# OpenHardware-Initiative/Drone-OA-IREE-ViT-Accelerator

Measured on AMD Instinct MI355X. Metric: frames/s on ITAViTLSTM int8, 60x90 depth input, higher is better.
Workload: dtype int8+f32; 1 GPU; ITAViTLSTM int8 end-to-end forward (BASELINE config 4): 1024 synthetic 60x90 depth frames per GPU per step, LSTM state carried, velocity all-gather; frames_per_gpu=1024, global_batch=1024, parallelism=dp1, image_dtype=u8, weights=seed-0 synthetic QAT (tests/golden), gather_every=1, gather=none (one GPU), schedule=one stream

## Files before the change

### drone-oa-iree-vit-accelerator_amd/csrc/ita_f16x3_kernels.h

```cpp
#pragma once
#include <type_traits>
#include "ita_device.h"

typedef _Float16 f16x8 __attribute__((ext_vector_type(8)));
typedef _Float16 f16x4 __attribute__((ext_vector_type(4)));
typedef float f32x16 __attribute__((ext_vector_type(16)));
typedef unsigned u32x2 __attribute__((ext_vector_type(2)));
typedef unsigned u32x4 __attribute__((ext_vector_type(4)));

__device__ __forceinline__ __amdgpu_buffer_rsrc_t ita_rsrc(const void* p) {
  return __builtin_amdgcn_make_buffer_rsrc(const_cast<void*>(p), (short)0, 0x7FFFFFFF, 0x00020000);
}
constexpr int ITA_SC1 = 16;

__device__ __forceinline__ void split_f16(float x, _Float16& hi, _Float16& lo) {
  hi = (_Float16)x;
  lo = (_Float16)(x - (float)hi);
}

struct ItaGemmSplitArgs {
  const _Float16 *a_hi, *a_lo; int lda;
  const _Float16 *w_hi, *w_lo; int ldw;
  float* out;
  int M, N, K;
// ... 51 lines not shown
  for (int i = 0; i < TM; ++i)
#pragma unroll
    for (int j = 0; j < TN; ++j)
#pragma unroll
      for (int e = 0; e < 16; ++e) acc[i][j][e] = 0.0f;

  auto stage = [&](int buf, int t) {
    char* b = lds + buf * L::BUF;
    const int k0 = kbeg + t * 64;
    const int m0s = (g.dbg & 16) ? 0 : m0, n0s = (g.dbg & 32) ? 0 : n0, k0s = (g.dbg & 64) ? t * 64 : k0;
    stage_plane<BM, NT>(g.a_hi, g.lda, m0s, g.M - 1, k0s, b, tid);
    stage_plane<BM, NT>(g.a_lo, g.lda, m0s, g.M - 1, k0s, b + L::A_PLANE, tid);
    stage_plane<BN, NT>(g.w_hi, g.ldw, n0s, g.N - 1, k0s, b + 2 * L::A_PLANE, tid);
    stage_plane<BN, NT>(g.w_lo, g.ldw, n0s, g.N - 1, k0s, b + 2 * L::A_PLANE + L::W_PLANE, tid);
  };

  auto compute = [&](int buf) {
    const char* b = lds + buf * L::BUF;
    const char *ah = b, *al = b + L::A_PLANE, *wh = b + 2 * L::A_PLANE, *wl = wh + L::W_PLANE;
#pragma unroll
    for (int ks = 0; ks < 4; ++ks) {
      f16x8 fah[TM], fal[TM], fwh[TN], fwl[TN];
#pragma unroll
      for (int i = 0; i < TM; ++i) {
        const int row = wm * (BM / WM) + i * 32 + r;
        fah[i] = frag_f16(ah, row, 2 * ks + h);
        fal[i] = frag_f16(al, row, 2 * ks + h);
      }
#pragma unroll
      for (int j = 0; j < TN; ++j) {
        const int row = wn * (BN / WN) + j * 32 + r;
        fwh[j] = frag_f16(wh, row, 2 * ks + h);
        fwl[j] = frag_f16(wl, row, 2 * ks + h);
      }
#pragma unroll
      for (int i = 0; i < TM; ++i)
#pragma unroll
        for (int j = 0; j < TN; ++j) {
          acc[i][j] = __builtin_amdgcn_mfma_f32_32x32x16_f16(fal[i], fwh[j], acc[i][j], 0, 0, 0);
          acc[i][j] = __builtin_amdgcn_mfma_f32_32x32x16_f16(fah[i], fwl[j], acc[i][j], 0, 0, 0);
          acc[i][j] = __builtin_amdgcn_mfma_f32_32x32x16_f16(fah[i], fwh[j], acc[i][j], 0, 0, 0);
        }
    }
  };
  int cur = 0;
  stage(0, 0);
  __syncthreads();
  for (int t = 0; t < nt; ++t) {
    if (t + 1 < nt && !(g.dbg & 2)) stage(cur ^ 1, t + 1);
    if (!(g.dbg & 1)) compute(g.dbg & 8 ? 0 : cur);
    if (!(g.dbg & 4)) __syncthreads();
    cur ^= 1;
  }
  float* out = g.out + (size_t)zsplit * g.M * g.N;
#pragma unroll
  for (int i = 0; i < TM; ++i)
#pragma unroll
    for (int j = 0; j < TN; ++j) {
      const int n = n0 + wn * (BN / WN) + j * 32 + r;
#pragma unroll
      for (int e = 0; e < 16; ++e) {
        const int m = m0 + wm * (BM / WM) + i * 32 + (e & 3) + 8 * (e >> 2) + 4 * h;
        if (m < g.M) __hip_atomic_store(out + (size_t)m * g.N + n, acc[i][j][e], __ATOMIC_RELAXED, __HIP_MEMORY_SCOPE_AGENT);
      }
    }
}

constexpr int ITA_GEMM_SMALL_NSTG = 3;
constexpr int ita_gemm_small_lds(int mt) { return ITA_GEMM_SMALL_NSTG * (2 * mt + 2) * 32 * 128; }
constexpr int ita_waitcnt_vm(int n) { return (n & 15) | ((n >> 4) << 14) | 0x0F70; }
template <int MT>
__global__ __launch_bounds__(256) void ita_gemm_f16x3_small_kernel(const ItaGemmSplitArgs g) {
  constexpr int NSTG = ITA_GEMM_SMALL_NSTG, PLANE = 32 * 128, APL = MT * PLANE, STG = 2 * APL + 2 * PLANE;
  constexpr int DMA = 2 * MT + 2;
  static_assert(NSTG == 3 && DMA < 64, "one younger k-tile in flight at the wait; vmcnt range");
  extern __shared__ __attribute__((aligned(16))) char lds[];
  const int tid = threadIdx.x, lane = tid & 63, wave = __builtin_amdgcn_readfirstlane(tid >> 6), r = lane & 31, h = lane >> 5;
  const int z = blockIdx.x % g.nsplit, n0 = (blockIdx.x / g.nsplit) * 32, m0 = blockIdx.y * 32 * MT;
  const int kslice = g.K / g.nsplit, kbeg = z * kslice, nt = kslice / 64;
  auto stage = [&](int kt, int slot) {
    char* b = lds + slot * STG;
    const int k0 = kbeg + kt * 64;
    stage_plane<32 * MT, 256>(g.a_hi, g.lda, m0, g.M - 1, k0, b, tid);
    stage_plane<32 * MT, 256>(g.a_lo, g.lda, m0, g.M - 1, k0, b + APL, tid);
    stage_plane<32, 256>(g.w_hi, g.ldw, n0, g.N - 1, k0, b + 2 * APL, tid);
    stage_plane<32, 256>(g.w_lo, g.ldw, n0, g.N - 1, k0, b + 2 * APL + PLANE, tid);
  };
#pragma unroll
  for (int s = 0; s < NSTG - 1; ++s)
    if (s < nt) stage(s, s);
  f32x16 acc;
#pragma unroll
  for (int e = 0; e < 16; ++e) acc[e] = 0.0f;
  const bool compute = wave < MT && m0 + 32 * wave < g.M;
  for (int kt = 0; kt < nt; ++kt) {
    if (kt + 1 < nt) __builtin_amdgcn_s_waitcnt(ita_waitcnt_vm(DMA)); else __builtin_amdgcn_s_waitcnt(ita_waitcnt_vm(0));
    __builtin_amdgcn_s_waitcnt(0xC07F);
    __builtin_amdgcn_s_barrier();
    asm volatile("" ::: "memory");
    __builtin_amdgcn_sched_barrier(0);
    if (kt + NSTG - 1 < nt) stage(kt + NSTG - 1, (kt + NSTG - 1) % NSTG);
    if (compute) {
      const char* b = lds + (kt % NSTG) * STG;
      const char *pah = b + wave * PLANE, *pal = b + APL + wave * PLANE, *pwh = b + 2 * APL, *pwl = pwh + PLANE;
#pragma unroll
      for (int ks = 0; ks < 4; ++ks) {
        const f16x8 ah = frag_f16(pah, r, 2 * ks + h), al = frag_f16(pal, r, 2 * ks + h);
        const f16x8 wh = frag_f16(pwh, r, 2 * ks + h), wl = frag_f16(pwl, r, 2 * ks + h);
        acc = __builtin_amdgcn_mfma_f32_32x32x16_f16(al, wh, acc, 0, 0, 0);
        acc = __builtin_amdgcn_mfma_f32_32x32x16_f16(ah, wl, acc, 0, 0, 0);
        acc = __builtin_amdgcn_mfma_f32_32x32x16_f16(ah, wh, acc, 0, 0, 0);
      }
    }
  }
  if (!compute) return;
  float* out = g.out + (size_t)z * g.M * g.N;
#pragma unroll
  for (int e = 0; e < 16; ++e) {
// ... 31 lines not shown
    }
  }
  float* out = g.out + (size_t)z * g.M * g.N;
#pragma unroll
  for (int e = 0; e < 16; ++e) {
    const int m = m0 + (e & 3) + 8 * (e >> 2) + 4 * h;
    if (m < g.M) out[(size_t)m * g.N + n0 + r] = acc[e];
  }
}

__device__ __forceinline__ size_t ita_lstm_plane_index(int b, int k) {
  return ((size_t)(((b >> 5) * 4 + (k >> 6)) * 4 + ((k >> 4) & 3)) * 64 + ((k >> 3) & 1) * 32 + (b & 31)) * 8 + (k & 7);
}
__device__ __forceinline__ float lstm_sigmoid_fast(float x) {
  return __builtin_amdgcn_rcpf(1.0f + __builtin_amdgcn_exp2f(x * -1.44269504088896341f));
}
__device__ __forceinline__ float lstm_tanh_fast(float x) {
  return 1.0f - 2.0f * __builtin_amdgcn_rcpf(__builtin_amdgcn_exp2f(x * 2.88539008177792681f) + 1.0f);
}
struct ItaLstmHeadArgs {
  const float* part; float inv_fold_scale;
  const _Float16 *w0_hi, *w0_lo; float inv_wscale0;
  const float* bias0;
  const _Float16 *w1_hi, *w1_lo, *w2_hi, *w2_lo;
  float inv_wscale1, inv_wscale2;
  const float *bsum1, *bsum2;
  const float *desvel, *quat;
  const float *h_in, *c_in;
  float *h_out, *c_out;
  size_t lstride;
  _Float16 *p1_hi, *p1_lo, *p2_hi, *p2_lo;
  const float *fc_w, *fc_b; float* vel;
  unsigned *cnt, *err;
  int B;
  const int* slots;
};
constexpr int ITA_HEAD_CNT_STRIDE = 64;
constexpr unsigned ITA_HEAD_ERR_TIMEOUT = 1;
constexpr unsigned long long ITA_HEAD_SPIN_TICKS = 200000000ull;
__device__ __forceinline__ f16x8 ita_load_sc1_f16x8(const _Float16* base, int byte_off) {
  return __builtin_bit_cast(f16x8, __builtin_amdgcn_raw_buffer_load_b128(ita_rsrc(base), byte_off, 0, ITA_SC1));
}
__device__ __forceinline__ bool ita_head_poll(unsigned* cnt, unsigned target, unsigned* err) {
  const unsigned long long t0 = wall_clock64();
  while (__hip_atomic_load(cnt, __ATOMIC_RELAXED, __HIP_MEMORY_SCOPE_AGENT) < target) {
    if (wall_clock64() - t0 > ITA_HEAD_SPIN_TICKS) {
      __hip_atomic_fetch_or(err, ITA_HEAD_ERR_TIMEOUT, __ATOMIC_RELAXED, __HIP_MEMORY_SCOPE_AGENT);
      return false;
    }
    __builtin_amdgcn_s_sleep(2);
  }
  return true;
}
template <int NS>
__global__ __launch_bounds__(256, 2) void ita_lstm_head_kernel(const ItaLstmHeadArgs a) {
  __shared__ __attribute__((aligned(16))) float big[32 * 132 + 32 * 36];
  __shared__ __attribute__((aligned(16))) f16x8 hin[2][2][4][2][64];
  __shared__ __attribute__((aligned(16))) _Float16 pub[2][32][8];
  __shared__ unsigned flag;
  float (*hs)[132] = (float (*)[132])big;
  float (*pt)[36] = (float (*)[36])(big + 32 * 132);
  float (*part)[16][64] = (float (*)[16][64])big;
  const int tid = threadIdx.x, lane = tid & 63, wave = __builtin_amdgcn_readfirstlane(tid >> 6);
  const int ft = blockIdx.x >> 4, ut = blockIdx.x & 15, f0 = ft * 32;
  const int r = lane & 31, h = lane >> 5;
  const int B = a.B;
  const int ef = tid >> 3, eu = tid & 7;
  int rh[4], rb0 = min(f0 + r, B - 1), reb = min(f0 + ef, B - 1);
#pragma unroll
  for (int i = 0; i < 4; ++i) rh[i] = min(f0 + 2 * (4 * wave + i) + h, B - 1);
  if (a.slots) {
#pragma unroll
    for (int i = 0; i < 4; ++i) rh[i] = a.slots[rh[i]];
    rb0 = a.slots[rb0];
    reb = a.slots[reb];
  }

  f32x4 pz[NS];
#pragma unroll
  for (int z = 0; z < NS; ++z)
    pz[z] = *(const f32x4*)(a.part + ((size_t)z * B + min(f0 + 8 * wave + (lane >> 3), B - 1)) * 512 + ut * 32 + 4 * (lane & 7));
  f32x4 hv[4];
#pragma unroll
  for (int i = 0; i < 4; ++i) hv[i] = *(const f32x4*)(a.h_in + (size_t)rh[i] * 128 + 4 * r);
  const int b0 = f0 + r, u0 = ut * 8 + 4 * h;
  const size_t sb0 = (size_t)rb0;
  if (wave >= 2) {
    f32x4 hx[2][4][2];
#pragma unroll
    for (int l = 0; l < 2; ++l)
#pragma unroll
      for (int s = 0; s < 4; ++s) {
        const float* src = a.h_in + (l + 1) * a.lstride + sb0 * 128 + 64 * (wave - 2) + 16 * s + 8 * h;
        hx[l][s][0] = *(const f32x4*)src;
        hx[l][s][1] = *(const f32x4*)(src + 4);
      }
    __builtin_amdgcn_sched_barrier(0);
#pragma unroll
    for (int l = 0; l < 2; ++l)
#pragma unroll
      for (int s = 0; s < 4; ++s) {
        f16x8 xh, xl;
#pragma unroll
        for (int j = 0; j < 8; ++j) {
          _Float16 hi, lo;
          split_f16(hx[l][s][j >> 2][j & 3], hi, lo);
          xh[j] = hi;
          xl[j] = lo;
        }
        hin[l][wave - 2][s][0][lane] = xh;
        hin[l][wave - 2][s][1][lane] = xl;
      }
  }
  f16x8 wh[9], wl[9];
  f32x4 q = {0.0f, 0.0f, 0.0f, 0.0f}, ci0 = {0.0f, 0.0f, 0.0f, 0.0f}, bz[4];
  float dv = 0.0f;
  if (wave == 0) {
    const _Float16* wfr_hi = a.w0_hi + ((size_t)ut * 9 * 64 + lane) * 8;
    const _Float16* wfr_lo = a.w0_lo + ((size_t)ut * 9 * 64 + lane) * 8;
#pragma unroll
    for (int s = 0; s < 9; ++s) {
      wh[s] = *(const f16x8*)(wfr_hi + s * 512);
      wl[s] = *(const f16x8*)(wfr_lo + s * 512);
    }
    const int bc = min(b0, B - 1);
    q = *(const f32x4*)(a.quat + (size_t)bc * 4);
    dv = a.desvel[bc];
    ci0 = *(const f32x4*)(a.c_in + sb0 * 128 + u0);
#pragma unroll
    for (int gt = 0; gt < 4; ++gt) bz[gt] = *(const f32x4*)(a.bias0 + gt * 128 + u0);
  }
  const size_t wo = ((size_t)((ut * 4 + wave) * 4) * 64 + lane) * 8;
  f16x8 w1h[4], w1l[4];
#pragma unroll
  for (int s = 0; s < 4; ++s) {
    w1h[s] = *(const f16x8*)(a.w1_hi + wo + 512 * s);
    w1l[s] = *(const f16x8*)(a.w1_lo + wo + 512 * s);
  }
  const int eb = f0 + ef, un = ut * 8 + eu;
  const size_t esb = (size_t)reb;
  const float c1_prev = a.c_in[a.lstride + esb * 128 + un], c2_prev = a.c_in[2 * a.lstride + esb * 128 + un];
  float bs1[4], bs2[4];
#pragma unroll
  for (int gt = 0; gt < 4; ++gt) {
    bs1[gt] = a.bsum1[gt * 128 + un];
    bs2[gt] = a.bsum2[gt * 128 + un];
  }
  __builtin_amdgcn_sched_barrier(0);
  {
    f32x4 ps = pz[0];
#pragma unroll
    for (int z = 1; z < NS; ++z) ps += pz[z];
    *(f32x4*)&pt[8 * wave + (lane >> 3)][4 * (lane & 7)] = ps;
  }
#pragma unroll
  for (int i = 0; i < 4; ++i) *(f32x4*)&hs[2 * (4 * wave + i) + h][4 * r] = hv[i];
  __syncthreads();

  f32x4 hn0 = {0.0f, 0.0f, 0.0f, 0.0f};
  if (wave == 0) {
    f32x16 acc;
#pragma unroll
    for (int e = 0; e < 16; ++e) acc[e] = 0.0f;
    f32x4 xlast0 = {0.0f, 0.0f, 0.0f, 0.0f};
    float xlast1 = 0.0f;
    if (h == 0) {
      xlast0 = (f32x4){dv / 10.0f, q.x, q.y, q.z};
      xlast1 = q.w;
    }
#pragma unroll
    for (int s = 0; s < 9; ++s) {
      f32x4 x0 = xlast0, x1 = {xlast1, 0.0f, 0.0f, 0.0f};
      if (s < 8) {
        x0 = *(const f32x4*)&hs[r][16 * s + 8 * h];
        x1 = *(const f32x4*)&hs[r][16 * s + 8 * h + 4];
      }
      f16x8 xh, xl;
#pragma unroll
      for (int j = 0; j < 8; ++j) {
        const float x = j < 4 ? x0[j & 3] : x1[j & 3];
        const _Float16 hi = (_Float16)x;
        xh[j] = hi;
        xl[j] = (_Float16)(x - (float)hi);
      }
      acc = __builtin_amdgcn_mfma_f32_32x32x16_f16(wl[s], xh, acc, 0, 0, 0);
      acc = __builtin_amdgcn_mfma_f32_32x32x16_f16(wh[s], xl, acc, 0, 0, 0);
      acc = __builtin_amdgcn_mfma_f32_32x32x16_f16(wh[s], xh, acc, 0, 0, 0);
    }
    f32x4 cn;
#pragma unroll
    for (int q = 0; q < 4; ++q) {
      float g[4];
#pragma unroll
      for (int gt = 0; gt < 4; ++gt)
        g[gt] = (pt[r][gt * 8 + 4 * h + q] * a.inv_fold_scale + acc[4 * gt + q] * a.inv_wscale0) + bz[gt][q];
      const float ig = lstm_sigmoid_fast(g[0]), fg = lstm_sigmoid_fast(g[1]), cg = lstm_tanh_fast(g[2]), og = lstm_sigmoid_fast(g[3]);
      const float c = fmaf(fg, ci0[q], ig * cg);
      cn[q] = c;
      hn0[q] = og * lstm_tanh_fast(c);
    }
    if (b0 < B) *(f32x4*)(a.c_out + sb0 * 128 + u0) = cn;
    f16x4 x_hi, x_lo;
#pragma unroll
    for (int q = 0; q < 4; ++q) {
      _Float16 x, y;
      split_f16(hn0[q], x, y); x_hi[q] = x; x_lo[q] = y;
    }
    const int o0 = (int)ita_lstm_plane_index(b0, u0) * 2;
    __builtin_amdgcn_raw_buffer_store_b64(__builtin_bit_cast(u32x2, x_hi), ita_rsrc(a.p1_hi), o0, 0, ITA_SC1);
    __builtin_amdgcn_raw_buffer_store_b64(__builtin_bit_cast(u32x2, x_lo), ita_rsrc(a.p1_lo), o0, 0, ITA_SC1);
  }
  asm volatile("s_waitcnt vmcnt(0)" ::: "memory");
  __syncthreads();
  if (tid == 0) __hip_atomic_fetch_add(a.cnt + ft * ITA_HEAD_CNT_STRIDE, 1u, __ATOMIC_RELAXED, __HIP_MEMORY_SCOPE_AGENT);
  f16x8 w2h[4], w2l[4];
#pragma unroll
  for (int s = 0; s < 4; ++s) {
    w2h[s] = *(const f16x8*)(a.w2_hi + wo + 512 * s);
    w2l[s] = *(const f16x8*)(a.w2_lo + wo + 512 * s);
  }

#pragma unroll
  for (int l = 1; l <= 2; ++l) {
    if (tid == 0) flag = ita_head_poll(a.cnt + ft * ITA_HEAD_CNT_STRIDE, 16u * l, a.err) ? 1u : 0u;
    __syncthreads();
    if (!flag) return;
    if (l == 1 && wave == 0 && b0 < B) *(f32x4*)(a.h_out + sb0 * 128 + u0) = hn0;
    f16x8 fah[4], fal[4];
    if (wave < 2) {
      const int ao = (((ft * 4 + wave) * 4) * 64 + lane) * 16;
      const _Float16* ph = l == 1 ? a.p1_hi : a.p2_hi;
      const _Float16* pl = l == 1 ? a.p1_lo : a.p2_lo;
#pragma unroll
      for (int s = 0; s < 4; ++s) {
        fah[s] = ita_load_sc1_f16x8(ph, ao + 1024 * s);
        fal[s] = ita_load_sc1_f16x8(pl, ao + 1024 * s);
      }
    } else {
#pragma unroll
      for (int s = 0; s < 4; ++s) {
        fah[s] = hin[l - 1][wave - 2][s][0][lane];
        fal[s] = hin[l - 1][wave - 2][s][1][lane];
      }
    }
    f32x16 acc;
#pragma unroll
    for (int e = 0; e < 16; ++e) acc[e] = 0.0f;
#pragma unroll
    for (int s = 0; s < 4; ++s) {
      const f16x8 fwh = l == 1 ? w1h[s] : w2h[s], fwl = l == 1 ? w1l[s] : w2l[s];
      acc = __builtin_amdgcn_mfma_f32_32x32x16_f16(fwl, fah[s], acc, 0, 0, 0);
      acc = __builtin_amdgcn_mfma_f32_32x32x16_f16(fwh, fal[s], acc, 0, 0, 0);
      acc = __builtin_amdgcn_mfma_f32_32x32x16_f16(fwh, fah[s], acc, 0, 0, 0);
    }
#pragma unroll
    for (int e = 0; e < 16; ++e) part[wave][e][lane] = acc[e];
    __syncthreads();
    float gsum[4];
    const int pl = ef + 32 * (eu >> 2);
#pragma unroll
    for (int gte = 0; gte < 4; ++gte) {
      const int e = 4 * gte + (eu & 3);
      gsum[gte] = ((part[0][e][pl] + part[1][e][pl]) + part[2][e][pl]) + part[3][e][pl];
    }
    const float iws = l == 1 ? a.inv_wscale1 : a.inv_wscale2;
    const float* bs = l == 1 ? bs1 : bs2;
    const float gi = gsum[0] * iws + bs[0], gf = gsum[1] * iws + bs[1], gg = gsum[2] * iws + bs[2], go = gsum[3] * iws + bs[3];
    const float ig = lstm_sigmoid_fast(gi), fg = lstm_sigmoid_fast(gf), cg = lstm_tanh_fast(gg), og = lstm_sigmoid_fast(go);
    const float c = fmaf(fg, l == 1 ? c1_prev : c2_prev, ig * cg);
    const float hn = og * lstm_tanh_fast(c);
    const size_t so = l * a.lstride + esb * 128 + un;
    if (eb < B) {
      a.c_out[so] = c;
      if (l == 1) a.h_out[so] = hn;
      else
        __builtin_amdgcn_raw_buffer_store_b32(__builtin_bit_cast(unsigned, hn), ita_rsrc(a.h_out), (int)(so * 4), 0, ITA_SC1);
    }
    if (l == 1) {
      _Float16 x, y;
      split_f16(hn, x, y);
      pub[0][ef][eu] = x;
      pub[1][ef][eu] = y;
      __syncthreads();
      if (wave == 0 && h == 0) {
        const int o = (int)ita_lstm_plane_index(f0 + r, ut * 8) * 2;
        const f16x8 vh = *(const f16x8*)&pub[0][r][0], vl = *(const f16x8*)&pub[1][r][0];
        __builtin_amdgcn_raw_buffer_store_b128(__builtin_bit_cast(u32x4, vh), ita_rsrc(a.p2_hi), o, 0, ITA_SC1);
        __builtin_amdgcn_raw_buffer_store_b128(__builtin_bit_cast(u32x4, vl), ita_rsrc(a.p2_lo), o, 0, ITA_SC1);
      }
    }
    asm volatile("s_waitcnt vmcnt(0)" ::: "memory");
    __syncthreads();
    if (tid == 0) {
      const unsigned prev = __hip_atomic_fetch_add(a.cnt + ft * ITA_HEAD_CNT_STRIDE, 1u, __ATOMIC_RELAXED, __HIP_MEMORY_SCOPE_AGENT);
      if (l == 2) flag = prev == 47u ? 1u : 0u;
    }
  }

  __syncthreads();
  if (!flag) return;
  if (tid == 0) __hip_atomic_store(a.cnt + ft * ITA_HEAD_CNT_STRIDE, 0u, __ATOMIC_RELAXED, __HIP_MEMORY_SCOPE_AGENT);
  float (*fw)[128] = (float (*)[128])(big + 32 * 132);
  int fro[4];
#pragma unroll
  for (int i = 0; i < 4; ++i) fro[i] = min(f0 + ((i * 256 + tid) >> 5), B - 1);
  if (a.slots) {
#pragma unroll
    for (int i = 0; i < 4; ++i) fro[i] = a.slots[fro[i]];
  }
  f32x4 hr[4];
#pragma unroll
  for (int i = 0; i < 4; ++i) {
    const int off = (int)((2 * a.lstride + (size_t)fro[i] * 128 + 4 * (tid & 31)) * 4);
    hr[i] = __builtin_bit_cast(f32x4, __builtin_amdgcn_raw_buffer_load_b128(ita_rsrc(a.h_out), off, 0, ITA_SC1));
  }
  const f32x4 wv = *(const f32x4*)(a.fc_w + 4 * min(tid, 95));
#pragma unroll
  for (int i = 0; i < 4; ++i) *(f32x4*)&hs[(i * 256 + tid) >> 5][4 * (tid & 31)] = hr[i];
  if (tid < 96) *(f32x4*)&fw[tid >> 5][4 * (tid & 31)] = wv;
  __syncthreads();
  if (tid < 96) {
    const int fr = tid / 3, o = tid - 3 * fr, b = f0 + fr;
    if (b < B) {
      float acc = a.fc_b[o];
      for (int k = 0; k < 128; ++k) acc = fmaf(hs[fr][k], fw[o][k], acc);
      a.vel[(size_t)b * 3 + o] = acc;
    }
  }
}

__global__ void ita_split_planes_kernel(const float* __restrict__ x, _Float16* __restrict__ hi, _Float16* __restrict__ lo,
                                        int width, int ld, int rows) {
  const size_t i8 = ((size_t)blockIdx.x * blockDim.x + threadIdx.x) * 8;
  if (i8 >= (size_t)rows * width) return;
  const size_t r = i8 / width, c = i8 - r * width;
  f16x8 vh, vl;
#pragma unroll
  for (int j = 0; j < 8; ++j) {
    _Float16 a, b;
    split_f16(x[i8 + j], a, b);
    vh[j] = a; vl[j] = b;
  }
  *(f16x8*)(hi + r * ld + c) = vh;
  *(f16x8*)(lo + r * ld + c) = vl;
}

__global__ void ita_impulse_kernel(float* x, int rows, int width, int col0) {
  const size_t idx = (size_t)blockIdx.x * blockDim.x + threadIdx.x;
  if (idx >= (size_t)rows * width) return;
  const int i = (int)(idx / width), c = (int)(idx % width);
  x[idx] = (c == col0 + i) ? 1.0f : 0.0f;
}

struct ItaTailBigArgs {
  const float* x;
  const _Float16 *w_hi, *w_lo;
  const float* bias;
  float inv_wscale;
  float* out;
  int B, E, TH, TW, CO, nchunk;
  int accumulate;
};
template <int NT, int WAVES, int TPS>
struct ItaTailBigLds {
  static constexpr int HP = (2 * WAVES + 2) * 34;
  static constexpr int A_PLANE = HP * 64;
  static constexpr int W_PLANE = TPS * NT * 16 * 64;
  static constexpr int AH = 0, AL = A_PLANE, WH = 2 * A_PLANE, WL = WH + W_PLANE;
  static constexpr int GEO_I = WL + W_PLANE;
  static constexpr int GEO_F = GEO_I + HP * 16;
  static constexpr int TOTAL = GEO_F + HP * 8;
};

template <int NT, int WAVES, int TPS>
__global__ __launch_bounds__(64 * WAVES) void ita_tail_big_kernel(const ItaTailBigArgs a) {
  using L = ItaTailBigLds<NT, WAVES, TPS>;
  static_assert(9 % TPS == 0, "taps per weight stage must divide 9");
  constexpr int W_CHUNK_HALVES = 9 * NT * 16 * 32;
  constexpr int NTHR = 64 * WAVES;
  extern __shared__ __attribute__((aligned(16))) char lds[];
  const int tid = threadIdx.x, lane = tid & 63, wave = tid >> 6;
// ... 484 lines not shown
```

### drone-oa-iree-vit-accelerator_amd/csrc/ita_stream_kernel.h

```cpp
#pragma once
#include "ita_int8_kernels.h"
#ifndef ITA_ABLATE
#define ITA_ABLATE 0
#endif

struct ItaStreamArgs {
  const char* image;
  const float* x;
  float* y;
  _Float16 *y_hi, *y_lo;
  int ld_planes;
  float* x1_tap;
  float inv_sx, mq, mk, mv, ml, mc, mo, so;
  float f_inv_sx, m1, m2, s2;
  int B;
  int fuse_ln;
  unsigned long long* stamps;
  const float* h0_src;
  float* h0_dst;
  const int* slots;
  const int8_t* xq;
  int8_t* yq;
  const void* img;
  float* tok_tap;
// ... 384 lines not shown
    const unsigned H1 = (unsigned)(8.0f * g.h1) & 7u, W1 = (unsigned)(32.0f * g.w1) & 31u, H0 = 8u - H1, W0 = 32u - W1;
    const unsigned w00 = (H0 * W0) & 255u, w01 = (H0 * W1) & 255u, w10 = (H1 * W0) & 255u, w11 = (H1 * W1) & 255u;
    __builtin_amdgcn_s_waitcnt(0xc07f);
    __builtin_amdgcn_wave_barrier();
    unsigned pb[13];
#pragma unroll
    for (int s = 0; s < 13; ++s) {
      if constexpr (ITA_ABLATE & 512) { pb[s] = w00 * s; continue; }
      const int off = tap[4 * s + kq];
      pb[s] = (unsigned)win[off] * w00 + (unsigned)win[off + 2] * w01 + (unsigned)win[off + 192] * w10 +
              (unsigned)win[off + 194] * w11;
    }
    tok_u8_fragments(pb, tk_a0, tk_a1);
  };
  auto tok_step = [&](int ct, int ol) {
    if constexpr (ITA_ABLATE & 1024) { tk_out[4 * ct] = __int_as_float(tk_a0[ct]); return; }
    float o4[4];
    tok_u8_tile<E>(lds + L::CW, ct, ol, ol >> 4, tk_a0, tk_a1, o4);
#pragma unroll
    for (int i = 0; i < 4; ++i) tk_out[4 * ct + i] = o4[i];
  };
  auto tok_finish = [&](int fb, bool store_tap, float (&xr)[EC], int ol) {
    const int qi = ol & 15, kq = ol >> 4, token = wave * 16 + qi;
#pragma unroll
    for (int i = 0; i < 16; ++i) xr[i] = tk_out[i];
    layernorm_q16<E>(xr, lnp + 4 * E, lnp + 5 * E, EC * kq);
    if (a.tok_tap && store_tap) {
      float* o = a.tok_tap + ((size_t)fb * S + token) * E + EC * kq;
#pragma unroll
      for (int i = 0; i < EC; i += 4) *(f32x4*)(o + i) = (f32x4){xr[i], xr[i + 1], xr[i + 2], xr[i + 3]};
    }
  };

  if (STAMP && a.stamps && (tid & 255) == 0)
    a.stamps[(((size_t)blockIdx.x * 8) * 2 + (wave >> 2)) * 16 + 12] = __builtin_amdgcn_s_memrealtime();
  float xr[EC];
  i32x4 xq_cur[NK];
  f32x4 h0_cur = {0.0f, 0.0f, 0.0f, 0.0f};
  int h0_row_next = 0;
  {
    int ol = lane;
    asm volatile("" : "+v"(ol));
    if constexpr (IO8) {
      const int8_t* xrow = a.xq + ((size_t)blockIdx.x * S + wave * 16 + (ol & 15)) * E + EC * (ol >> 4);
#pragma unroll
      for (int c = 0; c < NK; ++c) xq_cur[c] = *(const i32x4*)(xrow + 16 * c);
    } else if constexpr (TOK == 0) {
      ld_tok_items<E>(a.x + ((size_t)blockIdx.x * S + wave * 16 + (ol & 15)) * E, ol >> 4, xr);
    }
    if (a.h0_dst && tid < 32) {
      const size_t row = a.slots ? (size_t)a.slots[blockIdx.x] : (size_t)blockIdx.x;
      h0_cur = *(const f32x4*)(a.h0_src + row * 128 + 4 * tid);
    }
    constexpr int T0 = L::LNP / 16, NT = (L::IMAGE - L::LNP) / 16, NTJ = (NT + 511) / 512;
    constexpr int NW = L::LNP / 16, NWJ = (NW + 511) / 512;
    static_assert(L::LNP % 16 == 0, "");
    i32x4 vt[NTJ], vw[NWJ];
#pragma unroll
    for (int j = 0; j < NTJ; ++j) {
      const int p = tid + 512 * j;
      vt[j] = (i32x4){0, 0, 0, 0};
      if (p < NT) vt[j] = *(const i32x4*)(a.image + (size_t)(T0 + p) * 16);
    }
#pragma unroll
    for (int j = 0; j < NWJ; ++j) {
      const int p = tid + 512 * j;
      vw[j] = (i32x4){0, 0, 0, 0};
      if (p < NW) vw[j] = *(const i32x4*)(a.image + (size_t)p * 16);
    }
    if constexpr (TOK != 0) tok_fetch(blockIdx.x, ol);
    if (tid < 2 * P) colsum[tid] = ITA_ACC_BIAS;
#pragma unroll
    for (int j = 0; j < NTJ; ++j) {
      const int p = tid + 512 * j;
      if (p < NT) *(i32x4*)(lds + (T0 + p) * 16) = vt[j];
    }
#pragma unroll
    for (int j = 0; j < NWJ; ++j) {
      const int p = tid + 512 * j;
      if (p < NW) *(i32x4*)(lds + p * 16) = vw[j];
    }
    if constexpr (TOK != 0) tok_fill(ol);
    lds_barrier();
    if constexpr (TOK != 0) {
      tok_blend(ol);
#pragma unroll
      for (int ct = 0; ct < 4; ++ct) tok_step(ct, ol);
      tok_finish(blockIdx.x, true, xr, ol);
    }
    if constexpr (TOK == 0 && !IO8) tok_items_transpose<E>(xr);
  }
  if (STAMP && a.stamps && (tid & 255) == 0)
    a.stamps[(((size_t)blockIdx.x * 8) * 2 + (wave >> 2)) * 16 + 13] = __builtin_amdgcn_s_memrealtime();

  for (int b = blockIdx.x; b < a.B; b += gridDim.x, ++fi) {
    int ol = lane;
    asm volatile("" : "+v"(ol));
    const int qi = E > 64 ? (ol & 15) : qi0, kq = E > 64 ? (ol >> 4) : kq0, token = wave * 16 + qi;
    const int nb = b + gridDim.x;
    const bool more = nb < a.B;
    int* cs = colsum + (fi & 1) * P;
    ITA_SSTAMP(0);
    i32x4 xf[NK];
#pragma unroll
    for (int c = 0; c < NK; ++c) {
      if constexpr (IO8) {
        xf[c] = xq_cur[c];
      } else {
        unsigned p4[4];
        q_pack16(&xr[16 * c], a.inv_sx, p4);
        xf[c] = (i32x4){(int)p4[0], (int)p4[1], (int)p4[2], (int)p4[3]};
      }
    }
    if (!(ITA_ABLATE & 128) && a.h0_dst && tid < 32) {
      *(f32x4*)(a.h0_dst + (size_t)b * 128 + 4 * ol) = h0_cur;
      if (nb < a.B) h0_row_next = a.slots ? a.slots[nb] : nb;
    }

    i32x4 qf[3];
    {
      ItaFr<4 * NK> fr[2];
      i32x4 ac[3][4];
      auto load = [&](int g, ItaFr<4 * NK>& f, i32x4 (&acc)[4]) {
        const int mat = g / 3, t0 = 4 * (g - 3 * mat);
        if (mat == 0) ld_nat<NK, P>(f, acc, lds + L::WQ, l_bq, t0, qi, kq);
        else if (mat == 1) ld_nat<NK, P>(f, acc, lds + L::WK, l_bk, t0, qi, kq);
        else ld_natv<NK, P>(f, acc, lds + L::WV, (const int*)(lds + L::VB4), t0, qi, kq);
      };
      auto epilogue = [&](int g, const i32x4 (&acc)[4]) {
        const int mat = g / 3, gg = g - 3 * mat;
        if (mat == 0) {
          qf[gg] = rq_group(acc, a.mq, fq);
        } else if (mat == 1) {
          *(i32x4*)(lds + L::K + (((4 * gg + kq) * S + token) << 4)) = rq_group(acc, a.mk, fk);
        } else {
          const i32x4 p4 = rq_group(acc, a.mv, fv);
#pragma unroll
          for (int t = 0; t < 4; ++t) {
            const int d = (4 * gg + t) * 16 + qi;
            *(int*)(lds + L::VT + (((((wave >> 2) * 4 + kq) * P) + d) << 4) + 4 * (wave & 3)) = p4[t];
            atomicAdd(&cs[d], __builtin_amdgcn_sdot4(p4[t], 0x01010101, 0, false) << 7);
          }
// ... 385 lines not shown
```

### drone-oa-iree-vit-accelerator_amd/csrc/ita_plugin.hip

```cpp
#include <hip/hip_runtime.h>

#include <algorithm>
#include <cstdio>
#include <cstdlib>
#include <cstring>
#include <mutex>
#include <string>
#include <atomic>
#include <functional>
#include <thread>
#include <vector>

#include "../../include/ita_mi355x.h"
#include "../../include/ita_weights.h"
#include "../../include/ita_wire.h"
#include "ita_f16x3_kernels.h"
#include "ita_lstm_seq_kernel.h"
#include "ita_f32_kernels.h"
#include "ita_int8_kernels.h"
#include "ita_stream_kernel.h"
#include "ita_long_attn_kernel.h"
#include "ita_ffn_f32_kernel.h"
#include "ita_attn_f32_kernel.h"
#include "ita_ffn_f32_e128_kernel.h"
// ... 1206 lines not shown
  *status = 0;
  if (!h->head_sync) return ITA_OK;
  unsigned v = 0;
  HIPCHK(hipDeviceSynchronize());
  HIPCHK(hipMemcpy(&v, h->head_sync, sizeof(v), hipMemcpyDeviceToHost));
  if (v) {
    HIPCHK(hipMemset(h->head_sync, 0, h->head_sync_bytes));
    HIPCHK(hipDeviceSynchronize());
  }
  *status = (int)v;
  return ITA_OK;
}

int ita_get_attn_kind(ita_handle h, int layer, int* kind) {
  if (!h || !h->loaded) return fail(ITA_ERR_NO_WEIGHTS, "no weights loaded");
  if (!kind || layer < 0 || layer >= h->hdr.num_layers) return fail(ITA_ERR_INVALID_ARG, "bad pointer or layer");
  *kind = h->layers[layer].attn_f32 ? ITA_ATTN_F32 : ITA_ATTN_INT8;
  return ITA_OK;
}

int ita_mha_f32(ita_handle h, int layer, const float* x, float* y, int batch, void* stream) {
  int rc = check(h, batch);
  if (rc) return rc;
  if (!x || !y || layer < 0 || layer >= h->hdr.num_layers) return fail(ITA_ERR_INVALID_ARG, "bad pointer or layer");
  return launch_attn_f32(h, layer, x, y, batch, false, (hipStream_t)stream);
}

int ita_encoder_layer(ita_handle h, int layer, const float* x, float* y, int batch, void* stream) {
  int rc = check(h, batch);
  if (rc) return rc;
  if (!x || !y || layer < 0 || layer >= h->hdr.num_layers) return fail(ITA_ERR_INVALID_ARG, "bad pointer or layer");
  return launch_encoder(h, layer, x, y, nullptr, nullptr, nullptr, batch, (hipStream_t)stream);
}

int ita_debug_encoder_stamps(ita_handle h, int layer, const float* x, const void* image_u8, float* y, int batch,
                             unsigned long long* stamps, void* stream) {
  int rc = check(h, batch);
  if (rc) return rc;
  if ((!x && !image_u8) || !y || !stamps || layer < 0 || layer >= h->hdr.num_layers)
    return fail(ITA_ERR_INVALID_ARG, "bad argument");
  if (h->layers[layer].attn_f32) return fail(ITA_ERR_UNSUPPORTED, "this layer's attention is float32 (ITAW0003 blob): no stream kernel, no stamps");
  if (image_u8 ? !h->layers[layer].simg_tok : !h->layers[layer].simg_enc)
    return fail(ITA_ERR_UNSUPPORTED, "this layer does not run on the stream kernel");
  return launch_encoder(h, layer, x, y, nullptr, nullptr, nullptr, batch, (hipStream_t)stream, stamps, nullptr, nullptr,
                        nullptr, image_u8);
}

#ifdef ITA_UP_STAMP
int ita_debug_tail_up_stamps(unsigned long long* host_dst, int count) {
  if (hipDeviceSynchronize() != hipSuccess) return ITA_ERR_HIP;
  return hipMemcpyFromSymbol(host_dst, HIP_SYMBOL(ita_up_stamp_buf), sizeof(unsigned long long) * (size_t)count) == hipSuccess ? ITA_OK : ITA_ERR_HIP;
}
#endif
int ita_debug_softmax_rows(ita_handle h, const int8_t* logits, uint8_t* probs, int rows, void* stream) {
  int rc = check(h, rows, false);
  if (rc) return rc;
  if (!logits || !probs) return fail(ITA_ERR_INVALID_ARG, "null pointer");
  hipLaunchKernelGGL(ita_softmax_rows_kernel, dim3((rows + 15) / 16), dim3(64), 0, (hipStream_t)stream, logits, probs, rows);
  HIPCHK(hipGetLastError());
  return ITA_OK;
}

int ita_tokenizer(ita_handle h, const void* image, int image_dtype, float* tokens, int batch, void* stream) {
  int rc = check(h, batch);
  if (rc) return rc;
  if (!image || !tokens || (image_dtype != ITA_IMAGE_F32 && image_dtype != ITA_IMAGE_U8))
    return fail(ITA_ERR_INVALID_ARG, "bad pointer or image dtype");
  return launch_tokenizer(h, image, image_dtype, tokens, batch, (hipStream_t)stream);
}

int ita_fusion_tail(ita_handle h, const float* x, float* feat, int batch, void* stream) {
  int rc = check(h, batch);
  if (rc) return rc;
  if (!x || !feat) return fail(ITA_ERR_INVALID_ARG, "null pointer");
  return launch_tail(h, x, feat, 4608, batch, (hipStream_t)stream);
}

static void free_tail_large(ita_context* c) {
  if (c->tl_hi) (void)hipFree(c->tl_hi);
  if (c->tl_lo) (void)hipFree(c->tl_lo);
  if (c->tl_bias) (void)hipFree(c->tl_bias);
  if (c->tu_hi) (void)hipFree(c->tu_hi);
  if (c->tu_lo) (void)hipFree(c->tu_lo);
  if (c->ts_hi) (void)hipFree(c->ts_hi);
  if (c->ts_lo) (void)hipFree(c->ts_lo);
  c->tu_hi = c->tu_lo = c->ts_hi = c->ts_lo = nullptr;
  c->tl_hi = c->tl_lo = nullptr;
  c->tl_bias = nullptr;
  c->tl_E = c->tl_CO = c->tl_nt = c->tl_nchunk = 0;
}

int ita_fusion_tail_load(ita_handle h, const float* conv_w, const float* conv_b, int E, int out_ch) {
  int rc = check(h, 1, false);
  if (rc) return rc;
  if (!conv_w || !conv_b) return fail(ITA_ERR_INVALID_ARG, "null pointer");
  if (E <= 0 || E % 16 || out_ch <= 0 || out_ch > 64) return fail(ITA_ERR_UNSUPPORTED, "needs E % 16 == 0 and out_ch <= 64");
  free_tail_large(h);
  const int CIN = E / 4 + E, nchunk = (CIN + 31) / 32, nt = (out_ch + 15) / 16, cop = nt * 16;
  float mx = 0.0f;
  for (size_t i = 0; i < (size_t)out_ch * CIN * 9; ++i) mx = fabsf(conv_w[i]) > mx ? fabsf(conv_w[i]) : mx;
  int e = 0;
  if (mx > 0.0f) { int ex; frexpf(mx, &ex); e = 10 - ex; }
  const float sc = ldexpf(1.0f, e);
  std::vector<uint16_t> hi((size_t)nchunk * 9 * cop * 32, 0), lo(hi.size(), 0);
  for (int co = 0; co < out_ch; ++co)
    for (int c = 0; c < CIN; ++c)
// ... 607 lines not shown
```

Baseline: 11.32 million frames/s.

## Coalesce GEMM epilogue via LDS transpose and DMA stream-kernel weights into LDS

```diff
diff --git a/drone-oa-iree-vit-accelerator_amd/csrc/ita_f16x3_kernels.h b/drone-oa-iree-vit-accelerator_amd/csrc/ita_f16x3_kernels.h
--- a/drone-oa-iree-vit-accelerator_amd/csrc/ita_f16x3_kernels.h
+++ b/drone-oa-iree-vit-accelerator_amd/csrc/ita_f16x3_kernels.h
@@ -127,18 +127,40 @@
     if (!(g.dbg & 4)) __syncthreads();
     cur ^= 1;
   }
+  static_assert(WM * WN * TM * TN * 4096 <= L::TOTAL, "one 4 KB patch per 32 x 32 tile");
   float* out = g.out + (size_t)zsplit * g.M * g.N;
+  char* patch = lds + wave * (TM * TN * 4096);
 #pragma unroll
   for (int i = 0; i < TM; ++i)
 #pragma unroll
+    for (int j = 0; j < TN; ++j)
+#pragma unroll
+      for (int e = 0; e < 16; ++e)
+        *(float*)(patch + (i * TN + j) * 4096 + ((e & 3) + 8 * (e >> 2) + 4 * h) * 128 + r * 4) = acc[i][j][e];
+  asm volatile("" ::: "memory");
+  const int pr = lane >> 3, pc = lane & 7;
+  u32x4 v[TM][TN][4];
+#pragma unroll
+  for (int i = 0; i < TM; ++i)
+#pragma unroll
+    for (int j = 0; j < TN; ++j)
+#pragma unroll
+      for (int s = 0; s < 4; ++s) v[i][j][s] = *(const u32x4*)(patch + (i * TN + j) * 4096 + (8 * s + pr) * 128 + pc * 16);
+#pragma unroll
+  for (int i = 0; i < TM; ++i) {
+    const int mt = __builtin_amdgcn_readfirstlane(m0 + wm * (BM / WM) + i * 32);
+    if (mt >= g.M) continue;
+    const __amdgpu_buffer_rsrc_t ro = ita_rsrc(out + (size_t)mt * g.N);
+#pragma unroll
     for (int j = 0; j < TN; ++j) {
-      const int n = n0 + wn * (BN / WN) + j * 32 + r;
-#pragma unroll
-      for (int e = 0; e < 16; ++e) {
-        const int m = m0 + wm * (BM / WM) + i * 32 + (e & 3) + 8 * (e >> 2) + 4 * h;
-        if (m < g.M) __hip_atomic_store(out + (size_t)m * g.N + n, acc[i][j][e], __ATOMIC_RELAXED, __HIP_MEMORY_SCOPE_AGENT);
-      }
-    }
+      const int n = n0 + wn * (BN / WN) + j * 32 + 4 * pc;
+#pragma unroll
+      for (int s = 0; s < 4; ++s) {
+        const int ml = 8 * s + pr;
+        if (mt + ml < g.M) __builtin_amdgcn_raw_buffer_store_b128(v[i][j][s], ro, (ml * g.N + n) * 4, 0, ITA_SC1);
+      }
+    }
+  }
 }
 
 constexpr int ITA_GEMM_SMALL_NSTG = 3;
diff --git a/drone-oa-iree-vit-accelerator_amd/csrc/ita_stream_kernel.h b/drone-oa-iree-vit-accelerator_amd/csrc/ita_stream_kernel.h
--- a/drone-oa-iree-vit-accelerator_amd/csrc/ita_stream_kernel.h
+++ b/drone-oa-iree-vit-accelerator_amd/csrc/ita_stream_kernel.h
@@ -460,42 +460,48 @@
       const size_t row = a.slots ? (size_t)a.slots[blockIdx.x] : (size_t)blockIdx.x;
       h0_cur = *(const f32x4*)(a.h0_src + row * 128 + 4 * tid);
     }
-    constexpr int T0 = L::LNP / 16, NT = (L::IMAGE - L::LNP) / 16, NTJ = (NT + 511) / 512;
-    constexpr int NW = L::LNP / 16, NWJ = (NW + 511) / 512;
-    static_assert(L::LNP % 16 == 0, "");
-    i32x4 vt[NTJ], vw[NWJ];
+    constexpr int T0 = L::BIAS / 16, NT = (L::IMAGE - L::BIAS) / 16, NTJ = (NT + 511) / 512;
+    constexpr int NWJ = L::BIAS / (8 * 1024);
+    static_assert(L::BIAS % (8 * 1024) == 0, "every wave issues the same number of weight pieces: the counted wait below");
+    static_assert(NWJ < 64, "vmcnt range");
+    auto dma = [&](int piece0) {
+      __builtin_amdgcn_global_load_lds((const __attribute__((address_space(1))) void*)(a.image + (size_t)(piece0 + lane) * 16),
+                                       (__attribute__((address_space(3))) void*)(lds + piece0 * 16), 16, 0, 0);
+    };
 #pragma unroll
     for (int j = 0; j < NTJ; ++j) {
-      const int p = tid + 512 * j;
-      vt[j] = (i32x4){0, 0, 0, 0};
-      if (p < NT) vt[j] = *(const i32x4*)(a.image + (size_t)(T0 + p) * 16);
-    }
-#pragma unroll
-    for (int j = 0; j < NWJ; ++j) {
-      const int p = tid + 512 * j;
-      vw[j] = (i32x4){0, 0, 0, 0};
-      if (p < NW) vw[j] = *(const i32x4*)(a.image + (size_t)p * 16);
-    }
-    if constexpr (TOK != 0) tok_fetch(blockIdx.x, ol);
+      const int p0 = 64 * (wave + 8 * j);
+      if (p0 + lane < NT) dma(T0 + p0);
+    }
+    bool tk_ok[5] = {false, false, false, false, false};
+    if constexpr (TOK != 0) {
+      const TokGeo g = tok_geo(ol);
+      const uint8_t* src = (const uint8_t*)a.img + (size_t)blockIdx.x * 5400;
+      const int a0 = g.o & ~3;
+#pragma unroll
+      for (int j = 0; j < 5; ++j) {
+        const int aj = a0 + 4 * j;
+        tk_ok[j] = ol < 54 && g.row >= 0 && aj >= 0 && aj < 5400;
+        const uint8_t* pj = src + (tk_ok[j] ? aj : 0);
+        asm volatile("global_load_dword %0, %1, off" : "=v"(tk_d[j]) : "v"(pj) : "memory");
+      }
+    }
+#pragma unroll
+    for (int j = 0; j < NWJ; ++j) dma(64 * (wave + 8 * j));
     if (tid < 2 * P) colsum[tid] = ITA_ACC_BIAS;
-#pragma unroll
-    for (int j = 0; j < NTJ; ++j) {
-      const int p = tid + 512 * j;
-      if (p < NT) *(i32x4*)(lds + (T0 + p) * 16) = vt[j];
-    }
-#pragma unroll
-    for (int j = 0; j < NWJ; ++j) {
-      const int p = tid + 512 * j;
-      if (p < NW) *(i32x4*)(lds + p * 16) = vw[j];
-    }
-    if constexpr (TOK != 0) tok_fill(ol);
-    lds_barrier();
     if constexpr (TOK != 0) {
+      asm volatile("s_waitcnt vmcnt(%5)" : "+v"(tk_d[0]), "+v"(tk_d[1]), "+v"(tk_d[2]), "+v"(tk_d[3]), "+v"(tk_d[4]) : "n"(NWJ) : "memory");
+#pragma unroll
+      for (int j = 0; j < 5; ++j) tk_d[j] = tk_ok[j] ? tk_d[j] : 0u;
+      tok_fill(ol);
+      lds_barrier();
       tok_blend(ol);
 #pragma unroll
       for (int ct = 0; ct < 4; ++ct) tok_step(ct, ol);
       tok_finish(blockIdx.x, true, xr, ol);
     }
+    asm volatile("s_waitcnt vmcnt(0)" ::: "memory");
+    lds_barrier();
     if constexpr (TOK == 0 && !IO8) tok_items_transpose<E>(xr);
   }
   if (STAMP && a.stamps && (tid & 255) == 0)
```

After: 11.27 million frames/s. No clear change (-0.4%).

## Reorder LSTM head prologue loads and pre-split layer-0 inputs into swizzled LDS

Applied to the files above, without the earlier changes.

```diff
diff --git a/drone-oa-iree-vit-accelerator_amd/csrc/ita_f16x3_kernels.h b/drone-oa-iree-vit-accelerator_amd/csrc/ita_f16x3_kernels.h
--- a/drone-oa-iree-vit-accelerator_amd/csrc/ita_f16x3_kernels.h
+++ b/drone-oa-iree-vit-accelerator_amd/csrc/ita_f16x3_kernels.h
@@ -276,6 +276,13 @@
   }
   return true;
 }
+#ifdef ITA_HEAD_STAMP
+constexpr int ITA_HEAD_STAMP_WGS = 4096, ITA_HEAD_STAMP_N = 8;
+__device__ unsigned long long ita_head_stamp_buf[ITA_HEAD_STAMP_WGS * ITA_HEAD_STAMP_N];
+#define ITA_HEAD_ST(i) do { if (threadIdx.x == 0 && blockIdx.x < ITA_HEAD_STAMP_WGS) ita_head_stamp_buf[blockIdx.x * ITA_HEAD_STAMP_N + (i)] = __builtin_amdgcn_s_memrealtime(); } while (0)
+#else
+#define ITA_HEAD_ST(i) do { } while (0)
+#endif
 template <int NS>
 __global__ __launch_bounds__(256, 2) void ita_lstm_head_kernel(const ItaLstmHeadArgs a) {
   __shared__ __attribute__((aligned(16))) float big[32 * 132 + 32 * 36];
@@ -283,12 +290,18 @@
   __shared__ __attribute__((aligned(16))) _Float16 pub[2][32][8];
   __shared__ unsigned flag;
   float (*hs)[132] = (float (*)[132])big;
+  f16x8* xb = (f16x8*)big;
+  f16x4* xb4 = (f16x4*)big;
   float (*pt)[36] = (float (*)[36])(big + 32 * 132);
   float (*part)[16][64] = (float (*)[16][64])big;
   const int tid = threadIdx.x, lane = tid & 63, wave = __builtin_amdgcn_readfirstlane(tid >> 6);
   const int ft = blockIdx.x >> 4, ut = blockIdx.x & 15, f0 = ft * 32;
   const int r = lane & 31, h = lane >> 5;
   const int B = a.B;
+  ITA_HEAD_ST(0);
+#ifdef ITA_HEAD_STAMP
+  if (tid == 0 && blockIdx.x < ITA_HEAD_STAMP_WGS) ita_head_stamp_buf[blockIdx.x * ITA_HEAD_STAMP_N + 7] = 0;
+#endif
   const int ef = tid >> 3, eu = tid & 7;
   int rh[4], rb0 = min(f0 + r, B - 1), reb = min(f0 + ef, B - 1);
 #pragma unroll
@@ -309,17 +322,70 @@
   for (int i = 0; i < 4; ++i) hv[i] = *(const f32x4*)(a.h_in + (size_t)rh[i] * 128 + 4 * r);
   const int b0 = f0 + r, u0 = ut * 8 + 4 * h;
   const size_t sb0 = (size_t)rb0;
+  f16x8 wh[9], wl[9];
+  f32x4 q = {0.0f, 0.0f, 0.0f, 0.0f}, ci0 = {0.0f, 0.0f, 0.0f, 0.0f}, bz[4];
+  float dv = 0.0f;
+  const int eb = f0 + ef, un = ut * 8 + eu;
+  const size_t esb = (size_t)reb;
+  const float c1_prev = a.c_in[a.lstride + esb * 128 + un], c2_prev = a.c_in[2 * a.lstride + esb * 128 + un];
+  float bs1[4], bs2[4];
+#pragma unroll
+  for (int gt = 0; gt < 4; ++gt) {
+    bs1[gt] = a.bsum1[gt * 128 + un];
+    bs2[gt] = a.bsum2[gt * 128 + un];
+  }
+  const size_t wo = ((size_t)((ut * 4 + wave) * 4) * 64 + lane) * 8;
+  f16x8 w1h[4], w1l[4];
+  auto release_layer0 = [&]() {
+    __builtin_amdgcn_sched_barrier(0);
+    {
+      f32x4 ps = pz[0];
+#pragma unroll
+      for (int z = 1; z < NS; ++z) ps += pz[z];
+      *(f32x4*)&pt[8 * wave + (lane >> 3)][4 * (lane & 7)] = ps;
+    }
+#pragma unroll
+    for (int i = 0; i < 4; ++i) {
+      f16x4 xh, xl;
+#pragma unroll
+      for (int j = 0; j < 4; ++j) {
+        _Float16 hi, lo;
+        split_f16(hv[i][j], hi, lo);
+        xh[j] = hi;
+        xl[j] = lo;
+      }
+      const int fr = 2 * (4 * wave + i) + h;
+      xb4[(((r >> 1) * 32 + (fr ^ (r & 30))) << 1) + (r & 1)] = xh;
+      xb4[(((16 + (r >> 1)) * 32 + (fr ^ (r & 30))) << 1) + (r & 1)] = xl;
+    }
+    __syncthreads();
+    ITA_HEAD_ST(1);
+  };
+  auto load_w1 = [&]() {
+#pragma unroll
+    for (int s = 0; s < 4; ++s) {
+      w1h[s] = *(const f16x8*)(a.w1_hi + wo + 512 * s);
+      w1l[s] = *(const f16x8*)(a.w1_lo + wo + 512 * s);
+    }
+    __builtin_amdgcn_sched_barrier(0);
+  };
+
+  f32x4 hn0 = {0.0f, 0.0f, 0.0f, 0.0f};
   if (wave >= 2) {
     f32x4 hx[2][4][2];
-#pragma unroll
-    for (int l = 0; l < 2; ++l)
-#pragma unroll
-      for (int s = 0; s < 4; ++s) {
-        const float* src = a.h_in + (l + 1) * a.lstride + sb0 * 128 + 64 * (wave - 2) + 16 * s + 8 * h;
-        hx[l][s][0] = *(const f32x4*)src;
-        hx[l][s][1] = *(const f32x4*)(src + 4);
-      }
-    __builtin_amdgcn_sched_barrier(0);
+    auto load_hx = [&]() {
+#pragma unroll
+      for (int l = 0; l < 2; ++l)
+#pragma unroll
+        for (int s = 0; s < 4; ++s) {
+          const float* src = a.h_in + (l + 1) * a.lstride + sb0 * 128 + 64 * (wave - 2) + 16 * s + 8 * h;
+          hx[l][s][0] = *(const f32x4*)src;
+          hx[l][s][1] = *(const f32x4*)(src + 4);
+        }
+    };
+    load_hx();
+    release_layer0();
+    load_w1();
 #pragma unroll
     for (int l = 0; l < 2; ++l)
 #pragma unroll
@@ -335,108 +401,76 @@
         hin[l][wave - 2][s][0][lane] = xh;
         hin[l][wave - 2][s][1][lane] = xl;
       }
-  }
-  f16x8 wh[9], wl[9];
-  f32x4 q = {0.0f, 0.0f, 0.0f, 0.0f}, ci0 = {0.0f, 0.0f, 0.0f, 0.0f}, bz[4];
-  float dv = 0.0f;
-  if (wave == 0) {
-    const _Float16* wfr_hi = a.w0_hi + ((size_t)ut * 9 * 64 + lane) * 8;
-    const _Float16* wfr_lo = a.w0_lo + ((size_t)ut * 9 * 64 + lane) * 8;
-#pragma unroll
-    for (int s = 0; s < 9; ++s) {
-      wh[s] = *(const f16x8*)(wfr_hi + s * 512);
-      wl[s] = *(const f16x8*)(wfr_lo + s * 512);
-    }
-    const int bc = min(b0, B - 1);
-    q = *(const f32x4*)(a.quat + (size_t)bc * 4);
-    dv = a.desvel[bc];
-    ci0 = *(const f32x4*)(a.c_in + sb0 * 128 + u0);
-#pragma unroll
-    for (int gt = 0; gt < 4; ++gt) bz[gt] = *(const f32x4*)(a.bias0 + gt * 128 + u0);
-  }
-  const size_t wo = ((size_t)((ut * 4 + wave) * 4) * 64 + lane) * 8;
-  f16x8 w1h[4], w1l[4];
-#pragma unroll
-  for (int s = 0; s < 4; ++s) {
-    w1h[s] = *(const f16x8*)(a.w1_hi + wo + 512 * s);
-    w1l[s] = *(const f16x8*)(a.w1_lo + wo + 512 * s);
-  }
-  const int eb = f0 + ef, un = ut * 8 + eu;
-  const size_t esb = (size_t)reb;
-  const float c1_prev = a.c_in[a.lstride + esb * 128 + un], c2_prev = a.c_in[2 * a.lstride + esb * 128 + un];
-  float bs1[4], bs2[4];
-#pragma unroll
-  for (int gt = 0; gt < 4; ++gt) {
-    bs1[gt] = a.bsum1[gt * 128 + un];
-    bs2[gt] = a.bsum2[gt * 128 + un];
-  }
-  __builtin_amdgcn_sched_barrier(0);
-  {
-    f32x4 ps = pz[0];
-#pragma unroll
-    for (int z = 1; z < NS; ++z) ps += pz[z];
-    *(f32x4*)&pt[8 * wave + (lane >> 3)][4 * (lane & 7)] = ps;
-  }
-#pragma unroll
-  for (int i = 0; i < 4; ++i) *(f32x4*)&hs[2 * (4 * wave + i) + h][4 * r] = hv[i];
-  __syncthreads();
-
-  f32x4 hn0 = {0.0f, 0.0f, 0.0f, 0.0f};
-  if (wave == 0) {
-    f32x16 acc;
-#pragma unroll
-    for (int e = 0; e < 16; ++e) acc[e] = 0.0f;
-    f32x4 xlast0 = {0.0f, 0.0f, 0.0f, 0.0f};
-    float xlast1 = 0.0f;
-    if (h == 0) {
-      xlast0 = (f32x4){dv / 10.0f, q.x, q.y, q.z};
-      xlast1 = q.w;
-    }
-#pragma unroll
-    for (int s = 0; s < 9; ++s) {
-      f32x4 x0 = xlast0, x1 = {xlast1, 0.0f, 0.0f, 0.0f};
-      if (s < 8) {
-        x0 = *(const f32x4*)&hs[r][16 * s + 8 * h];
-        x1 = *(const f32x4*)&hs[r][16 * s + 8 * h + 4];
-      }
-      f16x8 xh, xl;
-#pragma unroll
+  } else {
+    if (wave == 0) {
+      const _Float16* wfr_hi = a.w0_hi + ((size_t)ut * 9 * 64 + lane) * 8;
+      const _Float16* wfr_lo = a.w0_lo + ((size_t)ut * 9 * 64 + lane) * 8;
+  #pragma unroll
+      for (int s = 0; s < 9; ++s) {
+        wh[s] = *(const f16x8*)(wfr_hi + s * 512);
+        wl[s] = *(const f16x8*)(wfr_lo + s * 512);
+      }
+      const int bc = min(b0, B - 1);
+      q = *(const f32x4*)(a.quat + (size_t)bc * 4);
+      dv = a.desvel[bc];
+      ci0 = *(const f32x4*)(a.c_in + sb0 * 128 + u0);
+  #pragma unroll
+      for (int gt = 0; gt < 4; ++gt) bz[gt] = *(const f32x4*)(a.bias0 + gt * 128 + u0);
+    }
+    release_layer0();
+    load_w1();
+    if (wave == 0) {
+      f32x16 acc;
+  #pragma unroll
+      for (int e = 0; e < 16; ++e) acc[e] = 0.0f;
+      f16x8 xh8, xl8;
+  #pragma unroll
       for (int j = 0; j < 8; ++j) {
-        const float x = j < 4 ? x0[j & 3] : x1[j & 3];
+        float x = 0.0f;
+        if (h == 0) x = j == 0 ? dv / 10.0f : j == 1 ? q.x : j == 2 ? q.y : j == 3 ? q.z : j == 4 ? q.w : 0.0f;
         const _Float16 hi = (_Float16)x;
-        xh[j] = hi;
-        xl[j] = (_Float16)(x - (float)hi);
-      }
-      acc = __builtin_amdgcn_mfma_f32_32x32x16_f16(wl[s], xh, acc, 0, 0, 0);
-      acc = __builtin_amdgcn_mfma_f32_32x32x16_f16(wh[s], xl, acc, 0, 0, 0);
-      acc = __builtin_amdgcn_mfma_f32_32x32x16_f16(wh[s], xh, acc, 0, 0, 0);
-    }
-    f32x4 cn;
-#pragma unroll
-    for (int q = 0; q < 4; ++q) {
-      float g[4];
-#pragma unroll
-      for (int gt = 0; gt < 4; ++gt)
-        g[gt] = (pt[r][gt * 8 + 4 * h + q] * a.inv_fold_scale + acc[4 * gt + q] * a.inv_wscale0) + bz[gt][q];
-      const float ig = lstm_sigmoid_fast(g[0]), fg = lstm_sigmoid_fast(g[1]), cg = lstm_tanh_fast(g[2]), og = lstm_sigmoid_fast(g[3]);
-      const float c = fmaf(fg, ci0[q], ig * cg);
-      cn[q] = c;
-      hn0[q] = og * lstm_tanh_fast(c);
-    }
-    if (b0 < B) *(f32x4*)(a.c_out + sb0 * 128 + u0) = cn;
-    f16x4 x_hi, x_lo;
-#pragma unroll
-    for (int q = 0; q < 4; ++q) {
-      _Float16 x, y;
-      split_f16(hn0[q], x, y); x_hi[q] = x; x_lo[q] = y;
-    }
-    const int o0 = (int)ita_lstm_plane_index(b0, u0) * 2;
-    __builtin_amdgcn_raw_buffer_store_b64(__builtin_bit_cast(u32x2, x_hi), ita_rsrc(a.p1_hi), o0, 0, ITA_SC1);
-    __builtin_amdgcn_raw_buffer_store_b64(__builtin_bit_cast(u32x2, x_lo), ita_rsrc(a.p1_lo), o0, 0, ITA_SC1);
+        xh8[j] = hi;
+        xl8[j] = (_Float16)(x - (float)hi);
+      }
+  #pragma unroll
+      for (int s = 0; s < 9; ++s) {
+        f16x8 xh = xh8, xl = xl8;
+        if (s < 8) {
+          xh = xb[(2 * s + h) * 32 + (r ^ (2 * (2 * s + h)))];
+          xl = xb[(16 + 2 * s + h) * 32 + (r ^ (2 * (2 * s + h)))];
+        }
+        acc = __builtin_amdgcn_mfma_f32_32x32x16_f16(wl[s], xh, acc, 0, 0, 0);
+        acc = __builtin_amdgcn_mfma_f32_32x32x16_f16(wh[s], xl, acc, 0, 0, 0);
+        acc = __builtin_amdgcn_mfma_f32_32x32x16_f16(wh[s], xh, acc, 0, 0, 0);
+      }
+      f32x4 cn;
+  #pragma unroll
+      for (int q = 0; q < 4; ++q) {
+        float g[4];
+  #pragma unroll
+        for (int gt = 0; gt < 4; ++gt)
+          g[gt] = (pt[r][gt * 8 + 4 * h + q] * a.inv_fold_scale + acc[4 * gt + q] * a.inv_wscale0) + bz[gt][q];
+        const float ig = lstm_sigmoid_fast(g[0]), fg = lstm_sigmoid_fast(g[1]), cg = lstm_tanh_fast(g[2]), og = lstm_sigmoid_fast(g[3]);
+        const float c = fmaf(fg, ci0[q], ig * cg);
+        cn[q] = c;
+        hn0[q] = og * lstm_tanh_fast(c);
+      }
+      if (b0 < B) *(f32x4*)(a.c_out + sb0 * 128 + u0) = cn;
+      f16x4 x_hi, x_lo;
+  #pragma unroll
+      for (int q = 0; q < 4; ++q) {
+        _Float16 x, y;
+        split_f16(hn0[q], x, y); x_hi[q] = x; x_lo[q] = y;
+      }
+      const int o0 = (int)ita_lstm_plane_index(b0, u0) * 2;
+      __builtin_amdgcn_raw_buffer_store_b64(__builtin_bit_cast(u32x2, x_hi), ita_rsrc(a.p1_hi), o0, 0, ITA_SC1);
+      __builtin_amdgcn_raw_buffer_store_b64(__builtin_bit_cast(u32x2, x_lo), ita_rsrc(a.p1_lo), o0, 0, ITA_SC1);
+    }
   }
   asm volatile("s_waitcnt vmcnt(0)" ::: "memory");
   __syncthreads();
   if (tid == 0) __hip_atomic_fetch_add(a.cnt + ft * ITA_HEAD_CNT_STRIDE, 1u, __ATOMIC_RELAXED, __HIP_MEMORY_SCOPE_AGENT);
+  ITA_HEAD_ST(2);
   f16x8 w2h[4], w2l[4];
 #pragma unroll
   for (int s = 0; s < 4; ++s) {
@@ -449,6 +483,7 @@
     if (tid == 0) flag = ita_head_poll(a.cnt + ft * ITA_HEAD_CNT_STRIDE, 16u * l, a.err) ? 1u : 0u;
     __syncthreads();
     if (!flag) return;
+    ITA_HEAD_ST(1 + 2 * l);
     if (l == 1 && wave == 0 && b0 < B) *(f32x4*)(a.h_out + sb0 * 128 + u0) = hn0;
     f16x8 fah[4], fal[4];
     if (wave < 2) {
@@ -519,6 +554,7 @@
       const unsigned prev = __hip_atomic_fetch_add(a.cnt + ft * ITA_HEAD_CNT_STRIDE, 1u, __ATOMIC_RELAXED, __HIP_MEMORY_SCOPE_AGENT);
       if (l == 2) flag = prev == 47u ? 1u : 0u;
     }
+    ITA_HEAD_ST(2 + 2 * l);
   }
 
   __syncthreads();
@@ -551,6 +587,7 @@
       a.vel[(size_t)b * 3 + o] = acc;
     }
   }
+  ITA_HEAD_ST(7);
 }
 
 __global__ void ita_split_planes_kernel(const float* __restrict__ x, _Float16* __restrict__ hi, _Float16* __restrict__ lo,
diff --git a/drone-oa-iree-vit-accelerator_amd/csrc/ita_plugin.hip b/drone-oa-iree-vit-accelerator_amd/csrc/ita_plugin.hip
--- a/drone-oa-iree-vit-accelerator_amd/csrc/ita_plugin.hip
+++ b/drone-oa-iree-vit-accelerator_amd/csrc/ita_plugin.hip
@@ -1282,6 +1282,12 @@
   return hipMemcpyFromSymbol(host_dst, HIP_SYMBOL(ita_up_stamp_buf), sizeof(unsigned long long) * (size_t)count) == hipSuccess ? ITA_OK : ITA_ERR_HIP;
 }
 #endif
+#ifdef ITA_HEAD_STAMP
+int ita_debug_head_stamps(unsigned long long* host_dst, int count) {
+  if (hipDeviceSynchronize() != hipSuccess) return ITA_ERR_HIP;
+  return hipMemcpyFromSymbol(host_dst, HIP_SYMBOL(ita_head_stamp_buf), sizeof(unsigned long long) * (size_t)count) == hipSuccess ? ITA_OK : ITA_ERR_HIP;
+}
+#endif
 int ita_debug_softmax_rows(ita_handle h, const int8_t* logits, uint8_t* probs, int rows, void* stream) {
   int rc = check(h, rows, false);
   if (rc) return rc;
```

Result: no change. 11.24 million frames/s before, 11.31 million frames/s after (median of 6 runs) (+0.7%).
